# imironhead/ml_super_resolution

Measured on AMD Instinct MI355X. Metric: VDSR-20 training patches/sec (41x41, batch 256 per GPU); fwd HR megapixels/sec alongside, higher is better.
Workload: dtype f32; 1 GPU; BASELINE configs[2]: VDSR 20-layer 3x3x64 residual, RGB, batch 256x41x41 per GPU, fwd+bwd+TF-Adam, random-init weights; global_batch=256, patch=41, parallelism=dp1

## Files before the change

### include/srx.h

```cpp
#ifndef SRX_H_
#define SRX_H_

#include <stddef.h>
#include <stdint.h>

#ifdef __cplusplus
extern "C" {
#endif

typedef void* srx_stream_t;

typedef enum {
    SRX_OK = 0,
    SRX_ERR_BAD_ARG = -1,
    SRX_ERR_UNSUPPORTED = -2,
    SRX_ERR_WORKSPACE = -3,
    SRX_ERR_LAUNCH = -4,
    SRX_ERR_ALIGN = -5
} srx_status;

typedef enum { SRX_PAD_SAME = 0, SRX_PAD_VALID = 1 } srx_pad_mode;

typedef enum {
    SRX_ACT_NONE = 0,
// ... 33 lines not shown

int srx_set_chain_fixed(int on);

int srx_conv2d_precision_supported(const srx_conv_desc* d, int op);

size_t srx_conv2d_workspace_bytes(const srx_conv_desc* d, int op);

int srx_conv2d_fwd(const srx_conv_desc* d, const float* x, const float* w, const float* bias,
                   const float* skip, float* y, void* ws, size_t ws_bytes, srx_stream_t stream);

int srx_conv2d_bwd_data(const srx_conv_desc* d, const float* dpre, const float* w,
                        const float* x_in, int in_act, float* dx_out, void* ws, size_t ws_bytes,
                        srx_stream_t stream);

int srx_conv2d_bwd_data_acc(const srx_conv_desc* d, const float* dpre, const float* w, const float* dx_acc,
                            float* dx_out, void* ws, size_t ws_bytes, srx_stream_t stream);

int srx_conv2d_bwd_filter(const srx_conv_desc* d, const float* x, const float* dpre, float* dw,
                          float* dbias, const float* w_for_decay, float wd_scale, void* ws,
                          size_t ws_bytes, srx_stream_t stream);

int srx_conv2d_bwd_filter_partials(const srx_conv_desc* d, const float* x, const float* dpre, void* ws,
                                   size_t ws_bytes, int* n_partials, srx_stream_t stream);
int srx_conv2d_bwd_filter_reduce(const srx_conv_desc* d, const void* ws, int n_partials, float* dw,
                                 float* dbias, const float* w_for_decay, float wd_scale,
                                 srx_stream_t stream);

int srx_conv2d_bwd_filter_batch(const srx_conv_desc* d, int n_layers, const float* const* x, const float* const* dpre,
                                float* const* dw, float* const* dbias, const float* const* w_for_decay, float wd_scale,
                                void* ws, size_t ws_bytes, srx_stream_t stream);
size_t srx_conv2d_bwd_filter_batch_workspace_bytes(const srx_conv_desc* d, int n_layers);
int srx_conv2d_bwd_filter_batch_plan(const srx_conv_desc* d, int n_layers, int* wgs_per_layer, int* grid);
int srx_set_wgrad_batch(int on);

int srx_act_bwd(const float* dy, const float* y, float* dpre, size_t numel, int act,
                srx_stream_t stream);

int srx_depth_to_space(const float* in, float* out, int N, int H, int W, int C, int r,
                       srx_stream_t stream);

int srx_stream_copy(const void* in, void* out, size_t bytes, srx_stream_t stream);

int srx_espcn_forward(const float* x, const float* w1, const float* b1, const float* w2, const float* b2,
                      const float* w3, const float* b3, float* hr, int N, int H, int W, int r,
                      srx_stream_t stream);
int srx_espcn_forward_keep(const float* x, const float* w1, const float* b1, const float* w2, const float* b2,
                           const float* w3, const float* b3, float* t1, float* t2, float* y, int N, int H, int W, int r,
                           srx_stream_t stream);

int srx_espcn_forward_u8(const uint8_t* lr, const float* lut, const float* w1, const float* b1, const float* w2,
                         const float* b2, const float* w3, const float* b3, uint8_t* hr, int N, int H, int W, int r,
                         srx_stream_t stream);
int srx_u8_lut_float(const uint8_t* in, const float* lut, float* out, size_t n, srx_stream_t stream);
int srx_unit_u8(const float* x, uint8_t* out, size_t n, srx_stream_t stream);

enum { SRX_YUV_BT601 = 0, SRX_YUV_BT709 = 1 };
typedef struct srx_yuv420_coeffs_t {
    int32_t yoff;
    int32_t cy, crv, cgu, cgv, cbu;
    int32_t kry, kgy, kby;
    int32_t kru, kgu, kbu, krv, kgv, kbv;
    int32_t reserved;
} srx_yuv420_coeffs_t;
int srx_yuv420_coeffs(int matrix, int full_range, srx_yuv420_coeffs_t* c);
int srx_yuv420_lut_float(const uint8_t* yuv, int N, int H, int W, const srx_yuv420_coeffs_t* c, const float* lut, float* out,
                         srx_stream_t stream);
// ... 315 lines not shown
```

### ml_super_resolution_amd/_lib.py

```python
import ctypes
import os

_HERE = os.path.dirname(os.path.abspath(__file__))
LIB_PATH = os.path.join(_HERE, 'libsrx.so')

SRX_OK = 0
PAD_SAME, PAD_VALID = 0, 1
ACT_NONE, ACT_RELU, ACT_TANH, ACT_LRELU, ACT_SIGMOID = 0, 1, 2, 3, 4
OP_FWD, OP_BWD_DATA, OP_BWD_FILTER = 0, 1, 2
PRECISION_FP32, PRECISION_BF16X3 = 0, 1
PRECISION_BY_NAME = {'highest': PRECISION_FP32, 'high': PRECISION_BF16X3}

ACT_BY_NAME = {None: ACT_NONE, 'none': ACT_NONE, 'relu': ACT_RELU, 'tanh': ACT_TANH,
               'lrelu': ACT_LRELU, 'leaky_relu': ACT_LRELU, 'sigmoid': ACT_SIGMOID}
PAD_BY_NAME = {'same': PAD_SAME, 'valid': PAD_VALID}

EXPORTS = [
    'srx_version', 'srx_last_error', 'srx_set_conv_path', 'srx_set_wgrad_path', 'srx_set_chain', 'srx_set_chain_fixed', 'srx_conv_chain', 'srx_conv_chain_supported', 'srx_conv2d_precision_supported', 'srx_conv2d_workspace_bytes', 'srx_conv2d_fwd',
    'srx_conv2d_bwd_data', 'srx_conv2d_bwd_filter', 'srx_conv2d_bwd_filter_partials', 'srx_conv2d_bwd_filter_reduce',
    'srx_conv2d_bwd_filter_batch', 'srx_conv2d_bwd_filter_batch_workspace_bytes', 'srx_conv2d_bwd_filter_batch_plan', 'srx_set_wgrad_batch', 'srx_act_bwd', 'srx_depth_to_space',
    'srx_space_to_depth', 'srx_stream_copy', 'srx_mse_fwd_bwd', 'srx_l2_loss', 'srx_reduce_scratch_bytes',
    'srx_adam_tf_step', 'srx_adam_tf_step_dev', 'srx_momentum_clip_step', 'srx_rownorm_loss_fwd_bwd', 'srx_psnr', 'srx_ssim', 'srx_ssim_scratch_bytes', 'srx_saturate_u8', 'srx_affine', 'srx_u8_to_unit_float', 'srx_gaussian_blur', 'srx_resize_bilinear',
    'srx_upsample_nearest', 'srx_upsample_nearest_bwd', 'srx_add_relu_grad',
    'srx_conv2d_bwd_data_acc', 'srx_conv3x3_blocked', 'srx_conv3x3_blocked_bwd_filter_workspace_bytes', 'srx_conv3x3_blocked_bwd_filter',
    'srx_conv3x3_blocked_ex', 'srx_conv3x3_blocked_bwd_filter_ex_workspace_bytes', 'srx_conv3x3_blocked_bwd_filter_ex',
    'srx_espcn_forward', 'srx_espcn_forward_keep', 'srx_debug_poison_lds', 'srx_srcnn_forward', 'srx_maxpool2x2', 'srx_maxpool2x2_bwd', 'srx_maxpool2x2_bwd_masked', 'srx_subsample2', 'srx_subsample2_bwd',
    'srx_channel_blocks_to_nhwc', 'srx_nhwc_to_channel_blocks', 'srx_channel_normalize', 'srx_channel_normalize_bwd',
    'srx_extract_patches16', 'srx_texture_gram', 'srx_texture_gram_bwd', 'srx_pil_resample_ksize', 'srx_pil_resample_coeffs', 'srx_resample_u8', 'srx_u8_to_pm1', 'srx_log_loss', 'srx_vgg_preprocess', 'srx_add_scaled', 'srx_resize_bicubic_tf', 'srx_column_sums', 'srx_gemm_workspace_bytes', 'srx_gemm', 'srx_gemm_route_of',
    'srx_feature_mosaic_u8', 'srx_summary_panel_bytes', 'srx_summary_panel_range_bytes', 'srx_summary_panel_u8', 'srx_summary_panel_range',
    'srx_vdsr_patch_table_check', 'srx_vdsr_patch_pairs',
    'srx_espcn_patch_table_check', 'srx_espcn_patch_pairs',
    'srx_espcn_eval_table_check', 'srx_espcn_eval_tiles', 'srx_espcn_eval_pairs',
    'srx_vdsr_eval_table_check', 'srx_vdsr_eval_tiles', 'srx_vdsr_eval_footprint', 'srx_vdsr_eval_pairs',
    'srx_enet_pairs_table_words', 'srx_enet_pairs_tables', 'srx_enet_patch_table_check', 'srx_enet_patch_pairs',
    'srx_enet_eval_coeff_words', 'srx_enet_eval_coeffs', 'srx_enet_eval_table_check', 'srx_enet_eval_tiles', 'srx_enet_eval_footprint',
    'srx_enet_eval_pairs',
    'srx_image_scores_scratch_bytes', 'srx_image_scores_plan', 'srx_image_scores_lds_bytes', 'srx_image_scores',
    'srx_dihedral_expand', 'srx_dihedral_merge',
    'srx_srcnn_pairs_band', 'srx_srcnn_pairs_lds_bytes', 'srx_srcnn_patch_table_check', 'srx_srcnn_patch_pairs',
    'srx_srcnn_eval_table_check', 'srx_srcnn_eval_tiles', 'srx_srcnn_eval_footprint', 'srx_srcnn_eval_pairs',
    'srx_espcn_forward_u8', 'srx_u8_lut_float', 'srx_unit_u8',
    'srx_yuv420_coeffs', 'srx_yuv420_lut_float', 'srx_unit_yuv420',
]


class SrxError(RuntimeError):
    pass


class ConvDesc(ctypes.Structure):
    _fields_ = [(n, ctypes.c_int32) for n in
                ('N', 'H', 'W', 'Cin', 'Cout', 'KH', 'KW', 'stride', 'pad_mode', 'act',
                 'post_add_relu', 'precision', 'subpixel_r')]
# ... 81 lines not shown
    global _lib
    if _lib is not None:
        return _lib
    if not os.path.exists(LIB_PATH):
        raise SrxError('libsrx.so not found at %s -- build it with `make -C %s` (or '
                       '__graft_entry__.build()); there is no CPU fallback' %
                       (LIB_PATH, os.path.join(_HERE, 'csrc')))
    import torch
    L = ctypes.CDLL(LIB_PATH)
    vp, sz, i, f = ctypes.c_void_p, ctypes.c_size_t, ctypes.c_int, ctypes.c_float
    dp = ctypes.POINTER(ConvDesc)
    L.srx_version.restype = ctypes.c_char_p
    L.srx_last_error.restype = ctypes.c_char_p
    L.srx_set_conv_path.argtypes = [i]
    L.srx_set_wgrad_path.argtypes = [i]
    L.srx_set_chain.argtypes = [i]
    L.srx_set_chain_fixed.argtypes = [i]
    L.srx_conv_chain_supported.argtypes = [dp, i, i]
    L.srx_conv_chain.argtypes = [dp, i, i, i, vp, vp, vp, vp, vp, vp]
    L.srx_conv2d_precision_supported.argtypes = [dp, i]
    L.srx_conv2d_workspace_bytes.argtypes = [dp, i]
    L.srx_conv2d_workspace_bytes.restype = sz
    L.srx_reduce_scratch_bytes.restype = sz
    L.srx_conv2d_fwd.argtypes = [dp, vp, vp, vp, vp, vp, vp, sz, vp]
    L.srx_conv2d_bwd_data.argtypes = [dp, vp, vp, vp, i, vp, vp, sz, vp]
    L.srx_conv2d_bwd_filter.argtypes = [dp, vp, vp, vp, vp, vp, f, vp, sz, vp]
    L.srx_conv2d_bwd_filter_partials.argtypes = [dp, vp, vp, vp, sz, ctypes.POINTER(ctypes.c_int), vp]
    L.srx_conv2d_bwd_filter_reduce.argtypes = [dp, vp, i, vp, vp, vp, f, vp]
    L.srx_conv2d_bwd_filter_batch.argtypes = [dp, i, vp, vp, vp, vp, vp, f, vp, sz, vp]
    L.srx_conv2d_bwd_filter_batch_workspace_bytes.argtypes = [dp, i]
    L.srx_conv2d_bwd_filter_batch_workspace_bytes.restype = sz
    L.srx_conv2d_bwd_filter_batch_plan.argtypes = [dp, i, ctypes.POINTER(ctypes.c_int), ctypes.POINTER(ctypes.c_int)]
    L.srx_set_wgrad_batch.argtypes = [i]
    L.srx_act_bwd.argtypes = [vp, vp, vp, sz, i, vp]
    L.srx_depth_to_space.argtypes = [vp, vp, i, i, i, i, i, vp]
    L.srx_space_to_depth.argtypes = [vp, vp, i, i, i, i, i, vp]
    L.srx_stream_copy.argtypes = [vp, vp, sz, vp]
    L.srx_mse_fwd_bwd.argtypes = [vp, vp, sz, f, vp, i, vp, vp, vp]
    L.srx_l2_loss.argtypes = [vp, vp, sz, f, vp, i, vp, vp]
    L.srx_adam_tf_step.argtypes = [vp, vp, vp, vp, sz, f, f, f, f, ctypes.c_int64, f, vp]
    L.srx_adam_tf_step_dev.argtypes = [vp, vp, vp, vp, sz, vp, f, f, f, f, vp]
    L.srx_momentum_clip_step.argtypes = [vp, vp, vp, sz, f, f, f, f, vp]
    L.srx_rownorm_loss_fwd_bwd.argtypes = [vp, vp, sz, sz, vp, vp, vp, vp]
    L.srx_psnr.argtypes = [vp, vp, vp, i, sz, f, vp]
    L.srx_ssim.argtypes = [vp, vp, vp, i, i, i, i, f, vp, vp]
    L.srx_ssim_scratch_bytes.argtypes = [i]
    L.srx_ssim_scratch_bytes.restype = sz
    sp, ip = ctypes.POINTER(ScoresDesc), ctypes.POINTER(ctypes.c_int)
    L.srx_image_scores_scratch_bytes.argtypes = [sp]
    L.srx_image_scores_scratch_bytes.restype = sz
    L.srx_image_scores_plan.argtypes = [sp, ip, ip, ip, ip]
    L.srx_image_scores_lds_bytes.argtypes = [sp]
    L.srx_image_scores_lds_bytes.restype = sz
    L.srx_image_scores.argtypes = [sp, vp, vp, vp, vp, vp]
    L.srx_dihedral_expand.argtypes = [vp, vp, vp, i, i, i, i, vp]
    L.srx_dihedral_merge.argtypes = [vp, vp, vp, i, i, i, i, vp]
    L.srx_saturate_u8.argtypes = [vp, vp, sz, vp]
    L.srx_feature_mosaic_u8.argtypes = [vp, vp, i, i, i, vp]
    L.srx_summary_panel_bytes.argtypes = [vp, i, i, i, i]
    L.srx_summary_panel_bytes.restype = sz
    L.srx_summary_panel_range_bytes.restype = sz
    L.srx_summary_panel_u8.argtypes = [vp, i, i, i, i, vp, vp, vp]
    L.srx_summary_panel_range.argtypes = [vp, i, i, i, i, vp, vp]
    L.srx_vdsr_patch_table_check.argtypes = [vp, i, i, sz]
    L.srx_vdsr_patch_pairs.argtypes = [vp, vp, i, i, vp, vp, vp]
    L.srx_espcn_patch_table_check.argtypes = [vp, i, i, i, sz]
# ... 92 lines not shown
```

### ml_super_resolution_amd/csrc/conv_inst_c4.hip

```cpp
#include "launchers.h"
namespace srx {
bool launch_conv_c4(const ConvKey& k, const ConvArgs& a, int grid, size_t lds, hipStream_t s, hipError_t* err) {
    SRX_CONV_CASE(3, 3, 4, 4, false, 2)
    SRX_CONV_CASE(3, 3, 4, 4, true, 2)
    SRX_CONV_CASE(3, 3, 4, 2, false, 2)
    SRX_CONV_CASE(3, 3, 4, 2, true, 2)
    SRX_CONV_CASE(3, 3, 4, 1, false, 2)
    SRX_CONV_CASE(5, 5, 4, 4, false, 2)
    SRX_CONV_CASE(5, 5, 4, 4, true, 2)
    SRX_CONV_CASE(5, 5, 4, 2, false, 2)
    SRX_CONV_CASE(5, 5, 4, 2, true, 2)
    SRX_CONV_CASE(9, 9, 4, 4, false, 2)
    SRX_CONV_CASE(9, 9, 4, 4, true, 2)
    return false;
}
}
```

### ml_super_resolution_amd/csrc/conv_narrow.hip

```cpp
#include "launchers.h"
namespace srx {
typedef float f32x3 __attribute__((ext_vector_type(3)));
typedef unsigned u32x3v __attribute__((ext_vector_type(3)));

template <int CTRL>
__device__ __forceinline__ float dpp_add(float v) {
    const int moved = __builtin_amdgcn_update_dpp(0, __float_as_int(v), CTRL, 0xf, 0xf, false);
    return v + __int_as_float(moved);
}

struct PixWalk {
    int n, oh, ow;
    __device__ __forceinline__ void init(unsigned p, int OH, int OW) {
        const unsigned t = p / (unsigned)OW;
        ow = (int)(p - t * (unsigned)OW);
        n = (int)(t / (unsigned)OH);
        oh = (int)(t - (unsigned)n * (unsigned)OH);
    }
    __device__ __forceinline__ void step16(int OH, int OW) { step(16, OH, OW); }
    __device__ __forceinline__ void step(int d, int OH, int OW) {
        ow += d;
        while (ow >= OW) {
            ow -= OW;
            oh += 1;
            if (oh == OH) { oh = 0; n += 1; }
        }
    }
};
template <int KH, int KW>
__device__ __forceinline__ void tap_offsets(int (&off)[KH * KW], const PixWalk& q, bool live, int H, int W, int pad_t, int pad_l,
                                            int PB, int lane_b) {
    const int centre = ((q.n * H + q.oh - pad_t) * W + (q.ow - pad_l)) * PB + lane_b;
    bool rok[KH], cok[KW];
#pragma unroll
    for (int kh = 0; kh < KH; ++kh) rok[kh] = live && (unsigned)(q.oh + kh - pad_t) < (unsigned)H;
#pragma unroll
    for (int kw = 0; kw < KW; ++kw) cok[kw] = (unsigned)(q.ow + kw - pad_l) < (unsigned)W;
#pragma unroll
    for (int kh = 0; kh < KH; ++kh)
#pragma unroll
        for (int kw = 0; kw < KW; ++kw)
            off[kh * KW + kw] = (rok[kh] && cok[kw]) ? centre + (kh * W + kw) * PB : kOobOffset;
}

template <int KH, int KW, int CIN, int CO>
__global__ __launch_bounds__(256) void conv_narrow_kernel(const ConvArgs a, long total_px, int iters) {
    static_assert(CIN == 64, "16 lanes x 4 channels per pixel");
    constexpr int TAPS = KH * KW;
    const int c4 = threadIdx.x & 15;
    const int sub = threadIdx.x >> 4;
    float wr[TAPS][4][CO];
#pragma unroll
    for (int t = 0; t < TAPS; ++t)
#pragma unroll
        for (int e = 0; e < 4; ++e)
#pragma unroll
            for (int c = 0; c < CO; ++c) wr[t][e][c] = a.w[((size_t)t * CIN + 4 * c4 + e) * CO + c];
    float bias[CO];
#pragma unroll
    for (int c = 0; c < CO; ++c) bias[c] = a.bias ? a.bias[c] : 0.0f;
    const __amdgpu_buffer_rsrc_t xrs = __builtin_amdgcn_make_buffer_rsrc(const_cast<float*>(a.x), 0,
                                                                         a.N * a.H * a.W * CIN * 4, 0x00020000);
    const unsigned p0 = blockIdx.x * (unsigned)iters * 16u + sub;
    PixWalk q;
    q.init(p0 < (unsigned)total_px ? p0 : 0u, a.OH, a.OW);
    for (int it = 0; it < iters; ++it, q.step16(a.OH, a.OW)) {
        const unsigned p = p0 + (unsigned)it * 16u;
        const bool live = p < (unsigned)total_px;
        int off[TAPS];
        tap_offsets<KH, KW>(off, q, live, a.H, a.W, a.pad_t, a.pad_l, CIN * 4, 16 * c4);
        f32x4 v[TAPS];
#pragma unroll
        for (int tp = 0; tp < TAPS; ++tp)
            v[tp] = __builtin_bit_cast(f32x4, __builtin_amdgcn_raw_buffer_load_b128(xrs, off[tp], 0, 0));
        float acc[CO];
// ... 87 lines not shown
        float r = acc[i];
#pragma unroll
        for (int o = LPP; o < 64; o <<= 1) r += __shfl_xor(r, o);
        if (sub % (64 / LPP) == 0) red[(wave * NV + i) * LPP + c4] = r;
    }
    __syncthreads();
    float* part = a.part + (size_t)blockIdx.x * a.part_stride;
    const int wn = TAPS * CW * CN;
    for (int q = threadIdx.x; q < NV * LPP; q += 256) {
        const int i = q / LPP, l = q % LPP;
        const float r = (red[(0 * NV + i) * LPP + l] + red[(1 * NV + i) * LPP + l]) +
                        (red[(2 * NV + i) * LPP + l] + red[(3 * NV + i) * LPP + l]);
        if (i < TAPS * 4 * CN) {
            int idx;
            if constexpr (NOUT) {
                const int c = i % CN, te = i / CN, e = te & 3, tp = te >> 2;
                idx = (tp * CW + 4 * l + e) * CN + c;
            } else {
                const int e = i & 3, tc = i >> 2;
                idx = tc * CW + 4 * l + e;
            }
            part[idx] = r;
        } else {
            const int b = i - TAPS * 4 * CN;
            if constexpr (NOUT) {
                if (l == 0) part[wn + b] = r;
            } else {
                part[wn + 4 * l + b] = r;
            }
        }
    }
}

bool launch_wgrad_narrow(const ConvKey& k, const WgradArgs& a, int grid, hipStream_t s, hipError_t* err) {
    if (k.kh != 3 || k.kw != 3) return false;
    const bool nout = a.Cin == 64 && a.Cout == 3, nin = a.Cin == 3 && a.Cout == 64, nin32 = a.Cin == 3 && a.Cout == 32;
    if (!nout && !nin && !nin32) return false;
    const long total = (long)a.N * a.OH * a.OW;
    if (total >= (1L << 31) - 4096 || (long)a.N * a.H * a.W * 64 * 4 >= (1L << 31) - 4096 || total * 64 * 4 >= (1L << 31) - 4096)
        return false;
    const long ppi = nin32 ? 32 : 16;
    const int iters = (int)((total + ppi * grid - 1) / (ppi * grid));
    if (nout)
        hipLaunchKernelGGL((wgrad_narrow_kernel<3, 3, true>), dim3(grid), dim3(256), 0, s, a, total, iters);
    else if (nin)
        hipLaunchKernelGGL((wgrad_narrow_kernel<3, 3, false>), dim3(grid), dim3(256), 0, s, a, total, iters);
    else
        hipLaunchKernelGGL((wgrad_narrow_kernel<3, 3, false, 32>), dim3(grid), dim3(256), 0, s, a, total, iters);
    *err = hipGetLastError();
    return true;
}

bool launch_conv_narrow(const ConvKey& k, const ConvArgs& a, hipStream_t s, hipError_t* err) {
    if (k.wt || a.Cout != 3 || a.mask) return false;
    if ((long)a.N * a.H * a.W * a.Cin * 4 >= (1L << 31) - 4096) return false;
    const long total = (long)a.N * a.OH * a.OW;
    int iters = 16;
    while (iters > 1 && total / (16L * iters) < 2048) iters >>= 1;
    const long blocks = (total + 16L * iters - 1) / (16L * iters);
    if (total >= (1L << 31) - 4096) return false;
    if (k.kh == 3 && k.kw == 3 && a.Cin == 64) {
        hipLaunchKernelGGL((conv_narrow_kernel<3, 3, 64, 3>), dim3((unsigned)blocks), dim3(256), 0, s, a, total, iters);
    } else {
        return false;
    }
    *err = hipGetLastError();
    return true;
}
}
```

### ml_super_resolution_amd/csrc/launchers.h

```cpp
#pragma once
#include "conv_kernels.hip.h"
#include "lds_launch.h"

namespace srx {

struct ConvKey {
    int kh, kw, cinp, nch;
    bool wt;
};

bool launch_conv_k3c64(const ConvKey& k, const ConvArgs& a, int grid, size_t lds, hipStream_t s, hipError_t* err);
bool launch_conv_k3c32(const ConvKey& k, const ConvArgs& a, int grid, size_t lds, hipStream_t s, hipError_t* err);
bool launch_conv_c4(const ConvKey& k, const ConvArgs& a, int grid, size_t lds, hipStream_t s, hipError_t* err);
bool launch_conv_misc(const ConvKey& k, const ConvArgs& a, int grid, size_t lds, hipStream_t s, hipError_t* err);
bool launch_pipe_k3c64(const ConvKey& k, const ConvArgs& a, int grid, size_t lds, hipStream_t s, hipError_t* err);
bool launch_pipe_other(const ConvKey& k, const ConvArgs& a, int grid, size_t lds, hipStream_t s, hipError_t* err);
bool launch_wgrad_narrow(const ConvKey& k, const WgradArgs& a, int grid, hipStream_t s, hipError_t* err);
bool launch_conv_narrow(const ConvKey& k, const ConvArgs& a, hipStream_t s, hipError_t* err);
bool launch_conv_1x1(const ConvKey& k, const ConvArgs& a, long min_pixels, hipStream_t s, hipError_t* err);
bool launch_conv_rows3x3(const ConvKey& k, const ConvArgs& a, long min_pixels, hipStream_t s, hipError_t* err);
bool launch_conv_pack3(const ConvKey& k, const ConvArgs& a, long min_pixels, hipStream_t s, hipError_t* err);
bool launch_conv_kwrows(const ConvKey& k, const ConvArgs& a, long min_pixels, hipStream_t s, hipError_t* err);
bool launch_pipe_strip(const ConvKey& k, const ConvArgs& a, int grid, size_t lds, hipStream_t s, hipError_t* err);
bool launch_conv_generic(const ConvKey& k, const ConvArgs& a, int grid, size_t lds, hipStream_t s, hipError_t* err);
bool launch_wgrad(const ConvKey& k, const WgradArgs& a, int grid, size_t lds, hipStream_t s, hipError_t* err);
bool launch_wgrad_generic(const ConvKey& k, const WgradArgs& a, int grid, size_t lds, hipStream_t s, hipError_t* err);
bool launch_wgrad_lin(const ConvKey& k, const WgradArgs& a, int grid, size_t lds, hipStream_t s, hipError_t* err);
bool launch_wgrad_lin_pack3(const ConvKey& k, const WgradArgs& a, int grid, size_t lds, hipStream_t s, hipError_t* err);
bool launch_wgrad_lin_strip(const ConvKey& k, const WgradArgs& a, int grid, size_t lds, hipStream_t s, hipError_t* err);
bool launch_wgrad_pipe(const ConvKey& k, const WgradArgs& a, int grid, size_t lds, hipStream_t s, hipError_t* err);
bool launch_wgrad_kwcols(const ConvKey& k, const WgradArgs& a, int max_partials, long min_pixels, int* n_partials, hipStream_t s, hipError_t* err);
bool launch_wgrad_1x1(const ConvKey& k, const WgradArgs& a, int max_partials, int* n_partials, hipStream_t s, hipError_t* err);
bool launch_wgrad_rows_full(const ConvKey& k, const WgradArgs& a, int grid, size_t lds, hipStream_t s, hipError_t* err);
bool launch_wgrad_rows_strip(const ConvKey& k, const WgradArgs& a, int grid, size_t lds, hipStream_t s, hipError_t* err);
bool launch_wgrad_lin_pairs(const ConvKey& k, const WgradPairs& q, int grid, int pairs, bool strips, size_t lds, hipStream_t s, hipError_t* err);

__attribute__((weak)) hipError_t launch_conv_chain(bool wt, bool aux, bool fixed, const ConvArgs& a, const ChainPtrs& c, int grid, size_t lds, hipStream_t s);

__attribute__((weak)) hipError_t launch_wgrad_rows_batch(const WgradArgs& a, const WgradBatchPtrs& c, int wpl, int layers, size_t lds, hipStream_t s);
__attribute__((weak)) hipError_t launch_wgrad_batch_reduce(const float* part, int wpl, int layers, int stride, int wn, int cout,
                                                           const WgradBatchOut& o, float wd, hipStream_t s);

// ... 82 lines not shown
```

### ml_super_resolution_amd/csrc/srx_api.hip

```cpp
#include <math.h>
#include <stdarg.h>
#include <atomic>
#include <stdio.h>
#include <stdlib.h>
#include <string.h>

#include "../../include/srx.h"
#include "elementwise.h"
#include "launchers.h"
#include "bf16x3.h"
#include "image_scores.h"
#include "dihedral.h"

using namespace srx;

namespace {

thread_local char g_err[512] = "";

struct Knobs {
    int pipe_default, narrow, wgrad_lin, wgrad_pipe, wgrad_pipe_strip, wgrad_rows_full, wgrad_1x1, wgrad_pack3, kwrows_min_pixels, big_route_min_pixels, strip_d2s, conv_1x1_min_pixels, pack3_dgrad;
    int chain, chain_fixed, wgrad_batch;
    unsigned long long* trace;
    int dbg;
};
int env_int(const char* name, int dflt) { const char* e = getenv(name); return e ? atoi(e) : dflt; }
Knobs read_knobs() {
    Knobs k;
    k.pipe_default = env_int("SRX_PIPE", 1);
    k.narrow = env_int("SRX_NARROW", 1);
    k.wgrad_lin = env_int("SRX_WGRAD_LIN", 1);
    k.wgrad_pipe = env_int("SRX_WGRAD_PIPE", 1);
    k.wgrad_pipe_strip = env_int("SRX_WGRAD_PIPE_STRIP", 1);
    k.kwrows_min_pixels = env_int("SRX_KWROWS_MIN_PIXELS", 4096);
    k.big_route_min_pixels = env_int("SRX_BIG_ROUTE_MIN_PIXELS", 60000);
    k.conv_1x1_min_pixels = env_int("SRX_CONV_1X1_MIN_PIXELS", 100000);
    k.pack3_dgrad = env_int("SRX_PACK3_DGRAD", 1);
    k.strip_d2s = env_int("SRX_STRIP_D2S", 1);
    k.wgrad_rows_full = env_int("SRX_WGRAD_ROWS_FULL", 1);
    k.wgrad_1x1 = env_int("SRX_WGRAD_1X1", 1);
    k.wgrad_pack3 = env_int("SRX_WGRAD_PACK3", 1);
    k.chain = env_int("SRX_CHAIN", 1);
    k.chain_fixed = env_int("SRX_CHAIN_FIXED", 1);
    k.wgrad_batch = env_int("SRX_WGRAD_BATCH", 1);
    k.trace = nullptr;
    k.dbg = 0;
#ifdef SRX_TRACE
    { const char* tp = getenv("SRX_TRACE_PTR"); k.trace = tp ? (unsigned long long*)strtoull(tp, nullptr, 0) : nullptr; }
    k.dbg = env_int("SRX_DBG", 0);
#endif
    return k;
}
const Knobs& knobs() { static const Knobs k = read_knobs(); return k; }

template <int (*Dflt)()>
struct Toggle {
    std::atomic<int> v{-1};
    int get() const { const int x = v.load(std::memory_order_relaxed); return x < 0 ? Dflt() : x; }
    int set(int x) { const int old = v.exchange(x, std::memory_order_relaxed); return old < 0 ? Dflt() : old; }
};
inline int on_off(int on) { return on < 0 ? -1 : (on ? 1 : 0); }
inline int pipe_default() { return knobs().pipe_default; }
inline int chain_default() { return knobs().chain ? 1 : 0; }
inline int chain_fixed_default() { return knobs().chain_fixed ? 1 : 0; }
inline int wgrad_batch_default() { return knobs().wgrad_batch ? 1 : 0; }
inline int wgrad_path_default() { return !knobs().wgrad_lin ? 0 : ((knobs().wgrad_pipe || knobs().wgrad_pipe_strip) ? 2 : 1); }
Toggle<pipe_default> g_use_pipe;
Toggle<chain_default> g_chain;
Toggle<chain_fixed_default> g_chain_fixed;
Toggle<wgrad_batch_default> g_wgrad_batch;
Toggle<wgrad_path_default> g_wgrad_path;
int use_pipe() { return g_use_pipe.get(); }
int wgrad_path() { return g_wgrad_path.get(); }

int cu_count() {
    static std::atomic<int> cached[64];
    int dev = 0;
    if (hipGetDevice(&dev) != hipSuccess || dev < 0 || dev >= 64) { (void)hipGetLastError(); return 256; }
    int n = cached[dev].load(std::memory_order_relaxed);
    if (n > 0) return n;
    if (hipDeviceGetAttribute(&n, hipDeviceAttributeMultiprocessorCount, dev) != hipSuccess || n <= 0) {
        (void)hipGetLastError();
        n = 256;
    }
    if (n > 256) n = 256;
    cached[dev].store(n, std::memory_order_relaxed);
    return n;
}

int fail(int code, const char* fmt, ...) {
    va_list ap;
    va_start(ap, fmt);
    vsnprintf(g_err, sizeof(g_err), fmt, ap);
    va_end(ap);
    return code;
}
int launch_status(hipError_t err, const char* what) {
    return err == hipSuccess ? SRX_OK : fail(SRX_ERR_LAUNCH, "%s: %s", what, hipGetErrorString(err));
}
}
namespace srx {
int set_error(int code, const char* fmt, ...) {
    va_list ap;
    va_start(ap, fmt);
    vsnprintf(g_err, sizeof(g_err), fmt, ap);
    va_end(ap);
    return code;
}
}
namespace {

inline bool aligned16(const void* p) { return (reinterpret_cast<uintptr_t>(p) & 15u) == 0; }

constexpr size_t kLdsBudget = 80 * 1024 - 336;
constexpr int kMaxGridLimit = 512;
inline int max_grid() { return 2 * cu_count(); }
inline int pipe_grid() { return cu_count(); }

struct Plan {
    int KH, KW, cinp, nch;
    int pad_t, pad_l, OH, OW;
    int TH, TW, NTX, RS;
    int units_total, grid;
    size_t lds_bytes;
};

size_t slot_bytes(int cinp) { return (size_t)((cinp == 4) ? 4 : cinp + 4) * 4; }
int pad_channels(int c) { return c <= 4 ? 4 : (c <= 32 ? 32 : (c <= 64 ? 64 : -1)); }
int chunks_for(int c) { return c <= 16 ? 1 : (c <= 32 ? 2 : (c <= 64 ? 4 : -1)); }

int make_plan(int N, int H, int W, int OH, int OW, int in_c, int out_c, int KH, int KW, int pad_t, int pad_l,
              Plan* p, bool lean_epilogue = true) {
    p->KH = KH; p->KW = KW;
    p->cinp = pad_channels(in_c);
// ... 611 lines not shown
    return srx_conv2d_bwd_filter_reduce(d, ws, n, dw, dbias, w_for_decay, wd_scale, stream);
}

namespace {
int wgrad_batch_plan(const srx_conv_desc* d, int layers, WgradArgs* a, int* wpl, int* grid, size_t* lds) {
    int rc = check_desc(d);
    if (rc) return rc;
    if (!g_wgrad_batch.get()) return fail(SRX_ERR_UNSUPPORTED, "bwd_filter_batch: switched off (srx_set_wgrad_batch / SRX_WGRAD_BATCH)");
    if (!launch_wgrad_rows_batch || !launch_wgrad_batch_reduce) return fail(SRX_ERR_UNSUPPORTED, "bwd_filter_batch: this build has no batch kernels");
    if (layers < 2 || layers > kChainMax) return fail(SRX_ERR_UNSUPPORTED, "bwd_filter_batch: %d layers (2..%d)", layers, kChainMax);
    if (d->precision != SRX_PRECISION_FP32) return fail(SRX_ERR_UNSUPPORTED, "bwd_filter_batch: precision %d (exact fp32 only)", d->precision);
    if (d->KH != 3 || d->KW != 3 || d->Cin != 64 || d->Cout != 64 || d->stride != 1 || d->pad_mode != SRX_PAD_SAME)
        return fail(SRX_ERR_UNSUPPORTED, "bwd_filter_batch: only 3x3 64->64 stride-1 SAME layers");
    if (d->W != 41) return fail(SRX_ERR_UNSUPPORTED, "bwd_filter_batch: W %d (only 41-pixel rows: wgrad_rows_full_kernel's shape)", d->W);
    const int wpath = wgrad_path();
    if (!wgrad_rows_full_switches(wpath))
        return fail(SRX_ERR_UNSUPPORTED, "bwd_filter_batch: the filter-gradient path is not wgrad_rows_full_kernel's (srx_set_wgrad_path)");
    LayerPlan lp;
    if ((rc = plan_layer(d, SRX_OP_BWD_FILTER, true, true, &lp)) != SRX_OK) return rc;
    if (!wgrad_rows_full_ok(d, lp, wpath)) return fail(SRX_ERR_UNSUPPORTED, "bwd_filter_batch: the shape is not on wgrad_rows_full_kernel's route");
    const long rows = (long)d->N * lp.OH;
    long w = pipe_grid() / layers;
    if (w > rows) w = rows;
    if (w < 1) return fail(SRX_ERR_UNSUPPORTED, "bwd_filter_batch: %d layers on a grid of %d", layers, pipe_grid());
    *wpl = (int)w;
    *grid = pipe_grid();
    fill_wgrad_args(a, d, lp);
    *lds = set_wgrad_rows_full_tile(a);
    return SRX_OK;
}
}

int srx_set_wgrad_batch(int on) { return g_wgrad_batch.set(on_off(on)); }

int srx_conv2d_bwd_filter_batch_plan(const srx_conv_desc* d, int n_layers, int* wgs_per_layer, int* grid) {
    WgradArgs a;
    int wpl = 0, g = 0;
    size_t lds;
    const int rc = wgrad_batch_plan(d, n_layers, &a, &wpl, &g, &lds);
    if (rc) { wpl = 0; g = 0; }
    if (wgs_per_layer) *wgs_per_layer = wpl;
    if (grid) *grid = g;
    return rc;
}

size_t srx_conv2d_bwd_filter_batch_workspace_bytes(const srx_conv_desc* d, int n_layers) {
    WgradArgs a;
    int wpl = 0, g = 0;
    size_t lds;
    if (wgrad_batch_plan(d, n_layers, &a, &wpl, &g, &lds) != SRX_OK) return 0;
    return partials_bytes(d, (size_t)n_layers * wpl);
}

int srx_conv2d_bwd_filter_batch(const srx_conv_desc* d, int n_layers, const float* const* x, const float* const* dpre, float* const* dw,
                                float* const* dbias, const float* const* w_for_decay, float wd_scale, void* ws, size_t ws_bytes,
                                srx_stream_t stream) {
    WgradArgs a;
    int wpl = 0, g = 0;
    size_t lds;
    int rc = wgrad_batch_plan(d, n_layers, &a, &wpl, &g, &lds);
    if (rc) return rc;
    if (!x || !dpre || !dw) return fail(SRX_ERR_BAD_ARG, "null pointer array");
    WgradBatchPtrs c;
    WgradBatchOut o;
    memset(&c, 0, sizeof(c));
    memset(&o, 0, sizeof(o));
// ... 413 lines not shown
```

### ml_super_resolution_amd/ops.py

```python
import ctypes
import os

import numpy as np
import torch

from . import _lib
from ._lib import ACT_BY_NAME, PAD_BY_NAME, ConvDesc, check
from ._lib import lib as _load_lib

_POISON_LDS = os.environ.get('SRX_POISON_LDS', '0') == '1'


def lib():
    L = _load_lib()
    if _POISON_LDS and torch.cuda.is_available():
        L.srx_debug_poison_lds(_stream())
    return L



def _stream():
    return ctypes.c_void_p(torch.cuda.current_stream().cuda_stream)


# ... 177 lines not shown
    return wpl.value, grid.value


def bwd_filter_batch_workspace_bytes(x_shape, w_shape, n_layers, padding='same', stride=1, precision='highest'):
    d = conv_desc(x_shape, w_shape, padding, stride=stride, precision=precision)
    return _load_lib().srx_conv2d_bwd_filter_batch_workspace_bytes(ctypes.byref(d), int(n_layers))


def conv2d_bwd_filter_batch(xs, dpres, dws, dbiases=None, w_for_decay=None, wd_scale=0.0, padding='same', workspace=None,
                            stride=1, precision='highest'):
    L = len(xs)
    if not (len(dpres) == len(dws) == L) or (dbiases is not None and len(dbiases) != L) or (w_for_decay is not None and len(w_for_decay) != L):
        raise ValueError('conv2d_bwd_filter_batch: the per-layer lists differ in length')
    for l in range(L):
        _chk(xs[l], 'x'); _chk(dpres[l], 'dpre'); _chk(dws[l], 'dw')
        _chk(None if dbiases is None else dbiases[l], 'dbias'); _chk(None if w_for_decay is None else w_for_decay[l], 'w_for_decay')
    d = conv_desc(xs[0].shape, dws[0].shape, padding, stride=stride, precision=precision)
    for l in range(L):
        if tuple(xs[l].shape) != tuple(xs[0].shape) or tuple(dpres[l].shape) != tuple(out_shape(d)) or tuple(dws[l].shape) != tuple(dws[0].shape):
            raise ValueError('conv2d_bwd_filter_batch: layer %d does not have the shape of layer 0' % l)
    if workspace is None:
        need = _load_lib().srx_conv2d_bwd_filter_batch_workspace_bytes(ctypes.byref(d), L)
        workspace = torch.empty((max(need, 16) + 3) // 4, dtype=torch.float32, device=xs[0].device)
    _chk(workspace, 'workspace')
    check(lib().srx_conv2d_bwd_filter_batch(ctypes.byref(d), L, _ptr_array(xs), _ptr_array(dpres), _ptr_array(dws),
                                            None if dbiases is None else _ptr_array(dbiases),
                                            None if w_for_decay is None else _ptr_array(w_for_decay), float(wd_scale),
                                            _ptr(workspace), workspace.numel() * 4, _stream()), 'srx_conv2d_bwd_filter_batch')
    return dws, dbiases


def set_wgrad_batch(on):
    return lib().srx_set_wgrad_batch(int(on))


def act_bwd(dy, y, act, out=None):
    _chk(dy, 'dy'); _chk(y, 'y')
    out = out if out is not None else torch.empty_like(dy)
    check(lib().srx_act_bwd(_ptr(dy), _ptr(y), _ptr(out), dy.numel(), ACT_BY_NAME[act], _stream()), 'srx_act_bwd')
    return out


def depth_to_space(x, r, out=None):
    _chk(x, 'x')
    N, H, W, D = x.shape
    if D % (r * r):
        raise ValueError('depth %d not divisible by r*r=%d' % (D, r * r))
    C = D // (r * r)
    out = out if out is not None else torch.empty((N, H * r, W * r, C), dtype=torch.float32, device=x.device)
    check(lib().srx_depth_to_space(_ptr(x), _ptr(out), N, H, W, C, r, _stream()), 'srx_depth_to_space')
    return out


def espcn_forward(x, params, r, out=None):
    _chk(x, 'x')
    for k, b in params:
        _chk(k, 'kernel'); _chk(b, 'bias')
    (w1, b1), (w2, b2), (w3, b3) = params
    N, H, W, C = x.shape
    if C != 3 or tuple(w1.shape) != (5, 5, 3, 64) or tuple(w2.shape) != (3, 3, 64, 32) or tuple(w3.shape) != (3, 3, 32, 3 * r * r):
        raise ValueError('espcn_forward: shapes do not describe ESPCN 5-3-3 with scaling factor %d' % r)
    out = out if out is not None else torch.empty((N, H * r, W * r, 3), dtype=torch.float32, device=x.device)
    check(lib().srx_espcn_forward(_ptr(x), _ptr(w1), _ptr(b1), _ptr(w2), _ptr(b2), _ptr(w3), _ptr(b3), _ptr(out),
                                  N, H, W, int(r), _stream()), 'srx_espcn_forward')
    return out

# ... 1269 lines not shown
```

Before: 20270 patches/s.

## Add MFMA streaming kernels for RGB first/last VDSR conv layers

Adds a streaming forward/dgrad kernel for 3x3 convolutions with 4-padded input channels and 64 outputs. It keeps weights in registers and uses 16x16x4 f32 MFMA with double-buffered buffer loads. It also adds an MFMA-based weight-gradient kernel for the narrow 3-channel layers, both input side and output side, with bias reduction through LDS. Both are enabled by default behind an SRX_RGB_STREAM toggle and aim to replace slower generic paths for the RGB edge layers. The risk is edge-case correctness, for example padding, masking and bias handling, and only modest gains, since these layers are a small part of VDSR-20.

```diff
diff --git a/include/srx.h b/include/srx.h
--- a/include/srx.h
+++ b/include/srx.h
@@ -89,6 +89,7 @@
 size_t srx_conv2d_bwd_filter_batch_workspace_bytes(const srx_conv_desc* d, int n_layers);
 int srx_conv2d_bwd_filter_batch_plan(const srx_conv_desc* d, int n_layers, int* wgs_per_layer, int* grid);
 int srx_set_wgrad_batch(int on);
+int srx_set_rgb_stream(int on);
 
 int srx_act_bwd(const float* dy, const float* y, float* dpre, size_t numel, int act,
                 srx_stream_t stream);
diff --git a/ml_super_resolution_amd/_lib.py b/ml_super_resolution_amd/_lib.py
--- a/ml_super_resolution_amd/_lib.py
+++ b/ml_super_resolution_amd/_lib.py
@@ -18,7 +18,7 @@
 EXPORTS = [
     'srx_version', 'srx_last_error', 'srx_set_conv_path', 'srx_set_wgrad_path', 'srx_set_chain', 'srx_set_chain_fixed', 'srx_conv_chain', 'srx_conv_chain_supported', 'srx_conv2d_precision_supported', 'srx_conv2d_workspace_bytes', 'srx_conv2d_fwd',
     'srx_conv2d_bwd_data', 'srx_conv2d_bwd_filter', 'srx_conv2d_bwd_filter_partials', 'srx_conv2d_bwd_filter_reduce',
-    'srx_conv2d_bwd_filter_batch', 'srx_conv2d_bwd_filter_batch_workspace_bytes', 'srx_conv2d_bwd_filter_batch_plan', 'srx_set_wgrad_batch', 'srx_act_bwd', 'srx_depth_to_space',
+    'srx_conv2d_bwd_filter_batch', 'srx_conv2d_bwd_filter_batch_workspace_bytes', 'srx_conv2d_bwd_filter_batch_plan', 'srx_set_wgrad_batch', 'srx_set_rgb_stream', 'srx_act_bwd', 'srx_depth_to_space',
     'srx_space_to_depth', 'srx_stream_copy', 'srx_mse_fwd_bwd', 'srx_l2_loss', 'srx_reduce_scratch_bytes',
     'srx_adam_tf_step', 'srx_adam_tf_step_dev', 'srx_momentum_clip_step', 'srx_rownorm_loss_fwd_bwd', 'srx_psnr', 'srx_ssim', 'srx_ssim_scratch_bytes', 'srx_saturate_u8', 'srx_affine', 'srx_u8_to_unit_float', 'srx_gaussian_blur', 'srx_resize_bilinear',
     'srx_upsample_nearest', 'srx_upsample_nearest_bwd', 'srx_add_relu_grad',
@@ -166,6 +166,7 @@
     L.srx_conv2d_bwd_filter_batch_workspace_bytes.restype = sz
     L.srx_conv2d_bwd_filter_batch_plan.argtypes = [dp, i, ctypes.POINTER(ctypes.c_int), ctypes.POINTER(ctypes.c_int)]
     L.srx_set_wgrad_batch.argtypes = [i]
+    L.srx_set_rgb_stream.argtypes = [i]
     L.srx_act_bwd.argtypes = [vp, vp, vp, sz, i, vp]
     L.srx_depth_to_space.argtypes = [vp, vp, i, i, i, i, i, vp]
     L.srx_space_to_depth.argtypes = [vp, vp, i, i, i, i, i, vp]
diff --git a/ml_super_resolution_amd/csrc/conv_inst_c4.hip b/ml_super_resolution_amd/csrc/conv_inst_c4.hip
--- a/ml_super_resolution_amd/csrc/conv_inst_c4.hip
+++ b/ml_super_resolution_amd/csrc/conv_inst_c4.hip
@@ -1,6 +1,119 @@
 #include "launchers.h"
+#include "pix_walk.h"
 namespace srx {
+namespace {
+
+constexpr int kStreamWaves = 4;
+
+constexpr int stream_wgs_per_cu(bool mask) { return mask ? 3 : 4; }
+
+template <bool MASK>
+__global__ __launch_bounds__(64 * kStreamWaves, stream_wgs_per_cu(MASK)) void conv_stream_c4_kernel(const ConvArgs a, int pixels, int wt) {
+    constexpr int TAPS = 9, NC = 4, CO = 64, DEPTH = 2;
+    const int lane = threadIdx.x & 63;
+    const int wave = __builtin_amdgcn_readfirstlane(threadIdx.x >> 6);
+    const int li = lane & 15, kq = lane >> 4;
+    const long steps_total = ((long)pixels + 15) >> 4;
+    const long gw = (long)blockIdx.x * kStreamWaves + wave, GW = (long)gridDim.x * kStreamWaves;
+    const int s0 = (int)(steps_total * gw / GW), nsteps = (int)(steps_total * (gw + 1) / GW) - s0;
+    const __amdgpu_buffer_rsrc_t xrs = __builtin_amdgcn_make_buffer_rsrc(const_cast<float*>(a.x), 0, a.N * a.H * a.W * a.Cin * 4, 0x00020000);
+    const __amdgpu_buffer_rsrc_t yrs = __builtin_amdgcn_make_buffer_rsrc(a.y, 0, pixels * CO * 4, 0x00020000);
+    const __amdgpu_buffer_rsrc_t mrs = __builtin_amdgcn_make_buffer_rsrc(const_cast<float*>(MASK ? a.mask : a.x), 0, MASK ? pixels * CO * 4 : 0, 0x00020000);
+
+    const bool kok = kq < a.Cin;
+    float wr[TAPS][NC];
+#pragma unroll
+    for (int tap = 0; tap < TAPS; ++tap)
+#pragma unroll
+        for (int c = 0; c < NC; ++c) {
+            const int co = 16 * c + li;
+            const int idx = wt ? ((TAPS - 1 - tap) * CO + co) * a.Cin + kq : (tap * a.Cin + kq) * CO + co;
+            const float v = a.w[kok ? idx : 0];
+            wr[tap][c] = kok ? v : 0.f;
+        }
+    f32x4 bias4[NC];
+#pragma unroll
+    for (int c = 0; c < NC; ++c) {
+        bias4[c] = f32x4{0.f, 0.f, 0.f, 0.f};
+        if (a.bias) bias4[c] = *reinterpret_cast<const f32x4*>(a.bias + 16 * c + 4 * kq);
+    }
+    const bool relu = a.act == ACT_RELU;
+
+    const int yoff = (li * CO + 4 * kq) * 4;
+    PixWalk q;
+    q.init((unsigned)(s0 * 16 + li < pixels ? s0 * 16 + li : 0), a.OH, a.OW);
+    float av[DEPTH][TAPS];
+    f32x4 mv[DEPTH][MASK ? NC : 1];
+    auto fetch = [&](int d, int s) {
+        const bool live = s < nsteps && (s0 + s) * 16 + li < pixels;
+        int off[TAPS];
+        tap_offsets<3, 3>(off, q, live && kok, a.H, a.W, a.pad_t, a.pad_l, a.Cin * 4, kq * 4);
+#pragma unroll
+        for (int tap = 0; tap < TAPS; ++tap)
+            av[d][tap] = __builtin_bit_cast(float, __builtin_amdgcn_raw_buffer_load_b32(xrs, off[tap], 0, 0));
+        if (MASK) {
+            const int mo = live ? yoff + (s0 + s) * (16 * CO * 4) : kOobOffset;
+#pragma unroll
+            for (int c = 0; c < NC; ++c) mv[d][c] = __builtin_bit_cast(f32x4, __builtin_amdgcn_raw_buffer_load_b128(mrs, mo, 64 * c, 0));
+        }
+        q.step16(a.OH, a.OW);
+    };
+#pragma unroll
+    for (int d = 0; d < DEPTH; ++d) fetch(d, d);
+    for (int s = 0; s < nsteps; s += DEPTH) {
+#pragma unroll
+        for (int d = 0; d < DEPTH; ++d) {
+            if (s + d >= nsteps) break;
+            float b[TAPS];
+            f32x4 m[MASK ? NC : 1];
+#pragma unroll
+            for (int tap = 0; tap < TAPS; ++tap) b[tap] = av[d][tap];
+            if (MASK) {
+#pragma unroll
+                for (int c = 0; c < NC; ++c) m[c] = mv[d][c];
+            }
+            fetch(d, s + d + DEPTH);
+            f32x4 acc[NC];
+#pragma unroll
+            for (int c = 0; c < NC; ++c) acc[c] = bias4[c];
+#pragma unroll
+            for (int tap = 0; tap < TAPS; ++tap)
+#pragma unroll
+                for (int c = 0; c < NC; ++c) acc[c] = __builtin_amdgcn_mfma_f32_16x16x4f32(wr[tap][c], b[tap], acc[c], 0, 0, 0);
+            const int so = ((s0 + s + d) * 16 + li < pixels) ? yoff + (s0 + s + d) * (16 * CO * 4) : kOobOffset;
+#pragma unroll
+            for (int c = 0; c < NC; ++c) {
+                f32x4 v = relu ? act_apply4(acc[c], ACT_RELU, 0.0f) : acc[c];
+                if (MASK) v = act_grad4(v, m[c], ACT_RELU, 0.0f);
+                __builtin_amdgcn_raw_buffer_store_b128(__builtin_bit_cast(u32x4v, v), yrs, so, 64 * c, 0);
+            }
+        }
+    }
+}
+
+bool launch_conv_stream_c4(const ConvKey& k, const ConvArgs& a, hipStream_t s, hipError_t* err) {
+    if (k.kh != 3 || k.kw != 3 || k.cinp != 4 || k.nch != 4) return false;
+    if (a.Cout != 64 || a.Cin < 1 || a.Cin > 4 || a.stride != 1 || a.skip || a.post_relu || a.d2s_r) return false;
+    if (!(a.act == ACT_NONE || a.act == ACT_RELU)) return false;
+    if (a.mask && (!k.wt || a.mask_act != ACT_RELU)) return false;
+    const long pixels = (long)a.N * a.OH * a.OW;
+    if (pixels < 1 || pixels * 64 * 4 >= (1L << 31) - 4096 || (long)a.N * a.H * a.W * a.Cin * 4 >= (1L << 31) - 4096) return false;
+    if (((uintptr_t)a.y | (uintptr_t)(a.mask ? a.mask : a.y) | (uintptr_t)(a.bias ? a.bias : a.y)) & 15u) return false;
+    const long steps = (pixels + 15) >> 4;
+    int grid = 256 * stream_wgs_per_cu(a.mask != nullptr);
+    if ((steps + kStreamWaves - 1) / kStreamWaves < grid) grid = (int)((steps + kStreamWaves - 1) / kStreamWaves);
+    if (a.mask)
+        hipLaunchKernelGGL((conv_stream_c4_kernel<true>), dim3(grid), dim3(64 * kStreamWaves), 0, s, a, (int)pixels, k.wt ? 1 : 0);
+    else
+        hipLaunchKernelGGL((conv_stream_c4_kernel<false>), dim3(grid), dim3(64 * kStreamWaves), 0, s, a, (int)pixels, k.wt ? 1 : 0);
+    *err = hipGetLastError();
+    return true;
+}
+
+}
+
 bool launch_conv_c4(const ConvKey& k, const ConvArgs& a, int grid, size_t lds, hipStream_t s, hipError_t* err) {
+    if (rgb_stream() && launch_conv_stream_c4(k, a, s, err)) return true;
     SRX_CONV_CASE(3, 3, 4, 4, false, 2)
     SRX_CONV_CASE(3, 3, 4, 4, true, 2)
     SRX_CONV_CASE(3, 3, 4, 2, false, 2)
diff --git a/ml_super_resolution_amd/csrc/conv_narrow.hip b/ml_super_resolution_amd/csrc/conv_narrow.hip
--- a/ml_super_resolution_amd/csrc/conv_narrow.hip
+++ b/ml_super_resolution_amd/csrc/conv_narrow.hip
@@ -1,4 +1,5 @@
 #include "launchers.h"
+#include "pix_walk.h"
 namespace srx {
 typedef float f32x3 __attribute__((ext_vector_type(3)));
 typedef unsigned u32x3v __attribute__((ext_vector_type(3)));
@@ -7,40 +8,6 @@
 __device__ __forceinline__ float dpp_add(float v) {
     const int moved = __builtin_amdgcn_update_dpp(0, __float_as_int(v), CTRL, 0xf, 0xf, false);
     return v + __int_as_float(moved);
-}
-
-struct PixWalk {
-    int n, oh, ow;
-    __device__ __forceinline__ void init(unsigned p, int OH, int OW) {
-        const unsigned t = p / (unsigned)OW;
-        ow = (int)(p - t * (unsigned)OW);
-        n = (int)(t / (unsigned)OH);
-        oh = (int)(t - (unsigned)n * (unsigned)OH);
-    }
-    __device__ __forceinline__ void step16(int OH, int OW) { step(16, OH, OW); }
-    __device__ __forceinline__ void step(int d, int OH, int OW) {
-        ow += d;
-        while (ow >= OW) {
-            ow -= OW;
-            oh += 1;
-            if (oh == OH) { oh = 0; n += 1; }
-        }
-    }
-};
-template <int KH, int KW>
-__device__ __forceinline__ void tap_offsets(int (&off)[KH * KW], const PixWalk& q, bool live, int H, int W, int pad_t, int pad_l,
-                                            int PB, int lane_b) {
-    const int centre = ((q.n * H + q.oh - pad_t) * W + (q.ow - pad_l)) * PB + lane_b;
-    bool rok[KH], cok[KW];
-#pragma unroll
-    for (int kh = 0; kh < KH; ++kh) rok[kh] = live && (unsigned)(q.oh + kh - pad_t) < (unsigned)H;
-#pragma unroll
-    for (int kw = 0; kw < KW; ++kw) cok[kw] = (unsigned)(q.ow + kw - pad_l) < (unsigned)W;
-#pragma unroll
-    for (int kh = 0; kh < KH; ++kh)
-#pragma unroll
-        for (int kw = 0; kw < KW; ++kw)
-            off[kh * KW + kw] = (rok[kh] && cok[kw]) ? centre + (kh * W + kw) * PB : kOobOffset;
 }
 
 template <int KH, int KW, int CIN, int CO>
@@ -194,6 +161,126 @@
     }
 }
 
+template <bool NOUT>
+__global__ __launch_bounds__(256, 2) void wgrad_narrow_mfma_kernel(const WgradArgs a, int total_px) {
+    constexpr int TAPS = 9, CW = 64, CN = 3, ROWS = TAPS * CN, DEPTH = 8;
+    constexpr int NV = 33;
+    __shared__ float red[4 * NV * 64];
+    const int lane = threadIdx.x & 63;
+    const int wave = __builtin_amdgcn_readfirstlane(threadIdx.x >> 6);
+    const int li = lane & 15, kq = lane >> 4;
+    const int WH = NOUT ? a.H : a.OH, WW = NOUT ? a.W : a.OW, NH = NOUT ? a.OH : a.H, NW = NOUT ? a.OW : a.W;
+    const __amdgpu_buffer_rsrc_t wrs = __builtin_amdgcn_make_buffer_rsrc(const_cast<float*>(NOUT ? a.x : a.dpre), 0, total_px * CW * 4, 0x00020000);
+    const __amdgpu_buffer_rsrc_t nrs = __builtin_amdgcn_make_buffer_rsrc(const_cast<float*>(NOUT ? a.dpre : a.x), 0, a.N * NH * NW * CN * 4, 0x00020000);
+    int dh[2], dw[2], cst[2];
+    bool rowok[2];
+#pragma unroll
+    for (int r = 0; r < 2; ++r) {
+        const int m = 16 * r + li, tap = m / CN, c = m - tap * CN, kh = tap / 3, kw = tap - kh * 3;
+        rowok[r] = m < ROWS;
+        dh[r] = NOUT ? a.pad_t - kh : kh - a.pad_t;
+        dw[r] = NOUT ? a.pad_l - kw : kw - a.pad_l;
+        cst[r] = ((dh[r] * NW + dw[r]) * CN + c) * 4;
+    }
+    const bool ones_lane = !NOUT && li == ROWS - 16;
+    const int tap_u = a.pad_t * 3 + a.pad_l;
+    const bool bsel0 = NOUT && li / CN == tap_u, bsel1 = NOUT && rowok[1] && (16 + li) / CN == tap_u;
+
+    const long steps_total = ((long)total_px + 3) >> 2;
+    const int s0 = (int)(steps_total * blockIdx.x / gridDim.x), nsteps = (int)(steps_total * (blockIdx.x + 1) / gridDim.x) - s0;
+    const int iters = nsteps > wave ? (nsteps - wave + 3) >> 2 : 0;
+    const int p0 = (s0 + wave) * 4 + kq;
+    PixWalk q;
+    q.init((unsigned)(p0 < total_px ? p0 : 0), WH, WW);
+    f32x4 bv[DEPTH];
+    float av[DEPTH][2], one[DEPTH];
+    auto fetch = [&](int d, int it) {
+        const int p = p0 + it * 16;
+        const bool live = (it < iters) & (p < total_px);
+        bv[d] = __builtin_bit_cast(f32x4, __builtin_amdgcn_raw_buffer_load_b128(wrs, live ? p * (CW * 4) + 16 * li : kOobOffset, 0, 0));
+        const int centre = ((q.n * NH + q.oh) * NW + q.ow) * (CN * 4);
+#pragma unroll
+        for (int r = 0; r < 2; ++r) {
+            const bool ok = live & rowok[r] & ((unsigned)(q.oh + dh[r]) < (unsigned)NH) & ((unsigned)(q.ow + dw[r]) < (unsigned)NW);
+            av[d][r] = __builtin_bit_cast(float, __builtin_amdgcn_raw_buffer_load_b32(nrs, ok ? centre + cst[r] : kOobOffset, 0, 0));
+        }
+        one[d] = live ? 1.0f : 0.0f;
+        q.step16(WH, WW);
+    };
+    f32x4 acc[2][4];
+#pragma unroll
+    for (int b = 0; b < 2; ++b)
+#pragma unroll
+        for (int i = 0; i < 4; ++i) acc[b][i] = f32x4{0.f, 0.f, 0.f, 0.f};
+    float bsum = 0.0f;
+#pragma unroll
+    for (int d = 0; d < DEPTH; ++d) fetch(d, d);
+    auto step = [&](int d, int it, bool refill) {
+        const f32x4 b = bv[d];
+        const float a0 = av[d][0];
+        const float a1 = ones_lane ? one[d] : av[d][1];
+#pragma unroll
+        for (int i = 0; i < 4; ++i) {
+            acc[0][i] = __builtin_amdgcn_mfma_f32_16x16x4f32(a0, b[i], acc[0][i], 0, 0, 0);
+            acc[1][i] = __builtin_amdgcn_mfma_f32_16x16x4f32(a1, b[i], acc[1][i], 0, 0, 0);
+        }
+        if (NOUT) {
+            const float sel = bsel0 ? a0 : (bsel1 ? a1 : 0.0f);
+            asm volatile("v_add_f32 %0, %0, %1" : "+v"(bsum) : "v"(sel));
+        }
+        __builtin_amdgcn_sched_barrier(0);
+        if (refill) fetch(d, it + DEPTH);
+    };
+    int it = 0;
+    for (; it + DEPTH <= iters; it += DEPTH) {
+#pragma unroll
+        for (int d = 0; d < DEPTH; ++d) step(d, it + d, true);
+    }
+#pragma unroll
+    for (int d = 0; d < DEPTH; ++d)
+        if (it + d < iters) step(d, it + d, false);
+#pragma unroll
+    for (int b = 0; b < 2; ++b)
+#pragma unroll
+        for (int i = 0; i < 4; ++i)
+#pragma unroll
+            for (int e = 0; e < 4; ++e) red[(wave * NV + (b * 4 + i) * 4 + e) * 64 + lane] = acc[b][i][e];
+    red[(wave * NV + 32) * 64 + lane] = bsum;
+    __syncthreads();
+    auto sum4 = [&](int v, int l) {
+        return (red[(0 * NV + v) * 64 + l] + red[(1 * NV + v) * 64 + l]) + (red[(2 * NV + v) * 64 + l] + red[(3 * NV + v) * 64 + l]);
+    };
+    float* part = a.part + (size_t)blockIdx.x * a.part_stride;
+    constexpr int wn = TAPS * CW * CN;
+    for (int idx = threadIdx.x; idx < wn + (NOUT ? 0 : CW); idx += 256) {
+        int m, ch;
+        if constexpr (NOUT) {
+            const int tap = idx / (CW * CN), rem = idx - tap * (CW * CN);
+            ch = rem / CN;
+            m = tap * CN + (rem - ch * CN);
+        } else {
+            m = idx >> 6;
+            ch = idx & 63;
+        }
+        part[idx] = sum4(((m >> 4) * 4 + (ch & 3)) * 4 + (m & 3), ((m & 15) >> 2) * 16 + (ch >> 2));
+    }
+    if (NOUT && threadIdx.x < CN) {
+        const int l = (tap_u * CN + threadIdx.x) & 15;
+        part[wn + threadIdx.x] = (sum4(32, l) + sum4(32, 16 + l)) + (sum4(32, 32 + l) + sum4(32, 48 + l));
+    }
+}
+
+bool launch_wgrad_narrow_mfma(const WgradArgs& a, bool nout, long total, int grid, hipStream_t s, hipError_t* err) {
+    if (nout && (a.pad_t < 0 || a.pad_t > 2 || a.pad_l < 0 || a.pad_l > 2 || a.OH > a.H || a.OW > a.W)) return false;
+    if (total < 1 || grid < 1) return false;
+    if (nout)
+        hipLaunchKernelGGL((wgrad_narrow_mfma_kernel<true>), dim3(grid), dim3(256), 0, s, a, (int)total);
+    else
+        hipLaunchKernelGGL((wgrad_narrow_mfma_kernel<false>), dim3(grid), dim3(256), 0, s, a, (int)total);
+    *err = hipGetLastError();
+    return true;
+}
+
 bool launch_wgrad_narrow(const ConvKey& k, const WgradArgs& a, int grid, hipStream_t s, hipError_t* err) {
     if (k.kh != 3 || k.kw != 3) return false;
     const bool nout = a.Cin == 64 && a.Cout == 3, nin = a.Cin == 3 && a.Cout == 64, nin32 = a.Cin == 3 && a.Cout == 32;
@@ -201,6 +288,7 @@
     const long total = (long)a.N * a.OH * a.OW;
     if (total >= (1L << 31) - 4096 || (long)a.N * a.H * a.W * 64 * 4 >= (1L << 31) - 4096 || total * 64 * 4 >= (1L << 31) - 4096)
         return false;
+    if (rgb_stream() && !nin32 && launch_wgrad_narrow_mfma(a, nout, nout ? (long)a.N * a.H * a.W : total, grid, s, err)) return true;
     const long ppi = nin32 ? 32 : 16;
     const int iters = (int)((total + ppi * grid - 1) / (ppi * grid));
     if (nout)
diff --git a/ml_super_resolution_amd/csrc/launchers.h b/ml_super_resolution_amd/csrc/launchers.h
--- a/ml_super_resolution_amd/csrc/launchers.h
+++ b/ml_super_resolution_amd/csrc/launchers.h
@@ -8,6 +8,8 @@
     int kh, kw, cinp, nch;
     bool wt;
 };
+
+int rgb_stream();
 
 bool launch_conv_k3c64(const ConvKey& k, const ConvArgs& a, int grid, size_t lds, hipStream_t s, hipError_t* err);
 bool launch_conv_k3c32(const ConvKey& k, const ConvArgs& a, int grid, size_t lds, hipStream_t s, hipError_t* err);
diff --git a/ml_super_resolution_amd/csrc/pix_walk.h b/ml_super_resolution_amd/csrc/pix_walk.h
--- /dev/null
+++ b/ml_super_resolution_amd/csrc/pix_walk.h
@@ -0,0 +1,40 @@
+#pragma once
+#include "conv_kernels.hip.h"
+
+namespace srx {
+
+struct PixWalk {
+    int n, oh, ow;
+    __device__ __forceinline__ void init(unsigned p, int OH, int OW) {
+        const unsigned t = p / (unsigned)OW;
+        ow = (int)(p - t * (unsigned)OW);
+        n = (int)(t / (unsigned)OH);
+        oh = (int)(t - (unsigned)n * (unsigned)OH);
+    }
+    __device__ __forceinline__ void step16(int OH, int OW) { step(16, OH, OW); }
+    __device__ __forceinline__ void step(int d, int OH, int OW) {
+        ow += d;
+        while (ow >= OW) {
+            ow -= OW;
+            oh += 1;
+            if (oh == OH) { oh = 0; n += 1; }
+        }
+    }
+};
+template <int KH, int KW>
+__device__ __forceinline__ void tap_offsets(int (&off)[KH * KW], const PixWalk& q, bool live, int H, int W, int pad_t, int pad_l,
+                                            int PB, int lane_b) {
+    const int centre = ((q.n * H + q.oh - pad_t) * W + (q.ow - pad_l)) * PB + lane_b;
+    bool rok[KH], cok[KW];
+#pragma unroll
+    for (int kh = 0; kh < KH; ++kh) rok[kh] = live && (unsigned)(q.oh + kh - pad_t) < (unsigned)H;
+#pragma unroll
+    for (int kw = 0; kw < KW; ++kw) cok[kw] = (unsigned)(q.ow + kw - pad_l) < (unsigned)W;
+#pragma unroll
+    for (int kh = 0; kh < KH; ++kh)
+#pragma unroll
+        for (int kw = 0; kw < KW; ++kw)
+            off[kh * KW + kw] = (rok[kh] && cok[kw]) ? centre + (kh * W + kw) * PB : kOobOffset;
+}
+
+}
diff --git a/ml_super_resolution_amd/csrc/srx_api.hip b/ml_super_resolution_amd/csrc/srx_api.hip
--- a/ml_super_resolution_amd/csrc/srx_api.hip
+++ b/ml_super_resolution_amd/csrc/srx_api.hip
@@ -20,7 +20,7 @@
 
 struct Knobs {
     int pipe_default, narrow, wgrad_lin, wgrad_pipe, wgrad_pipe_strip, wgrad_rows_full, wgrad_1x1, wgrad_pack3, kwrows_min_pixels, big_route_min_pixels, strip_d2s, conv_1x1_min_pixels, pack3_dgrad;
-    int chain, chain_fixed, wgrad_batch;
+    int chain, chain_fixed, wgrad_batch, rgb_stream;
     unsigned long long* trace;
     int dbg;
 };
@@ -43,6 +43,7 @@
     k.chain = env_int("SRX_CHAIN", 1);
     k.chain_fixed = env_int("SRX_CHAIN_FIXED", 1);
     k.wgrad_batch = env_int("SRX_WGRAD_BATCH", 1);
+    k.rgb_stream = env_int("SRX_RGB_STREAM", 1);
     k.trace = nullptr;
     k.dbg = 0;
 #ifdef SRX_TRACE
@@ -64,12 +65,14 @@
 inline int chain_default() { return knobs().chain ? 1 : 0; }
 inline int chain_fixed_default() { return knobs().chain_fixed ? 1 : 0; }
 inline int wgrad_batch_default() { return knobs().wgrad_batch ? 1 : 0; }
+inline int rgb_stream_default() { return knobs().rgb_stream ? 1 : 0; }
 inline int wgrad_path_default() { return !knobs().wgrad_lin ? 0 : ((knobs().wgrad_pipe || knobs().wgrad_pipe_strip) ? 2 : 1); }
 Toggle<pipe_default> g_use_pipe;
 Toggle<chain_default> g_chain;
 Toggle<chain_fixed_default> g_chain_fixed;
 Toggle<wgrad_batch_default> g_wgrad_batch;
 Toggle<wgrad_path_default> g_wgrad_path;
+Toggle<rgb_stream_default> g_rgb_stream;
 int use_pipe() { return g_use_pipe.get(); }
 int wgrad_path() { return g_wgrad_path.get(); }
 
@@ -100,6 +103,7 @@
 }
 }
 namespace srx {
+int rgb_stream() { return g_rgb_stream.get(); }
 int set_error(int code, const char* fmt, ...) {
     va_list ap;
     va_start(ap, fmt);
@@ -777,6 +781,7 @@
 }
 
 int srx_set_wgrad_batch(int on) { return g_wgrad_batch.set(on_off(on)); }
+int srx_set_rgb_stream(int on) { return g_rgb_stream.set(on_off(on)); }
 
 int srx_conv2d_bwd_filter_batch_plan(const srx_conv_desc* d, int n_layers, int* wgs_per_layer, int* grid) {
     WgradArgs a;
diff --git a/ml_super_resolution_amd/ops.py b/ml_super_resolution_amd/ops.py
--- a/ml_super_resolution_amd/ops.py
+++ b/ml_super_resolution_amd/ops.py
@@ -233,6 +233,10 @@
 
 def set_wgrad_batch(on):
     return lib().srx_set_wgrad_batch(int(on))
+
+
+def set_rgb_stream(on):
+    return lib().srx_set_rgb_stream(int(on))
 
 
 def act_bwd(dy, y, act, out=None):
```

Measured after the change: 20400 patches/s (median of 6 runs). Within noise of the previous version (+0.6%).
